# DarlingHang/st-nerf

Measured on NVIDIA H100. Metric: rays/sec, higher is better.
Workload: dtype f32 via fp16x3 split products (wgmma), f32 accumulate

## Files before the change

### st-nerf_b200/csrc/mlp_tc.cu

```cuda
#include <cuda_fp16.h>
#include <string.h>
#include <type_traits>
#include <vector>
#include "mlp_tc.cuh"
#include "resample.cuh"

namespace stnerf {

namespace {

constexpr int TILE_M = 128;
constexpr int ABLOCK = 16384;
constexpr int STAGE_BYTES = 16384;
constexpr int NTHREADS = 384;
constexpr int MATH_WG0 = 1, N_MATH_WARPS = 8;
constexpr int MAX_STAGE = 8;
constexpr int REGS_WG0 = 56, REGS_MATH = 224;
static_assert(128 * REGS_WG0 + 256 * REGS_MATH <= 384 * 168, "register file");
constexpr int BAR_WFULL = 0, BAR_WEMPTY = 8, BAR_RAWFULL = 16, BAR_RAWEMPTY = 18;
constexpr int MISC_ROWS = 256;
constexpr int MISC_PART = MISC_ROWS + 128 * 24;
constexpr int MISC_CDF = MISC_PART + 2048;
constexpr int MISC_TOTAL = MISC_CDF + 512;

__device__ __forceinline__ uint32_t smem_u32(const void* p) { return (uint32_t)__cvta_generic_to_shared(p); }

__device__ __forceinline__ void mbar_init(uint32_t bar, uint32_t count) {
  asm volatile("mbarrier.init.shared::cta.b64 [%0], %1;" ::"r"(bar), "r"(count) : "memory");
}
__device__ __forceinline__ void mbar_arrive(uint32_t bar) {
  asm volatile("mbarrier.arrive.shared::cta.b64 _, [%0];" ::"r"(bar) : "memory");
}
__device__ __forceinline__ void mbar_arrive_if(uint32_t bar, bool pred) {
  asm volatile("{\n\t.reg .pred p;\n\tsetp.ne.b32 p, %1, 0;\n\t@p mbarrier.arrive.shared::cta.b64 _, [%0];\n\t}" ::"r"(bar), "r"((uint32_t)pred)
               : "memory");
}
__device__ __forceinline__ void mbar_expect_tx(uint32_t bar, uint32_t bytes) {
  asm volatile("mbarrier.arrive.expect_tx.shared::cta.b64 _, [%0], %1;" ::"r"(bar), "r"(bytes) : "memory");
}
__device__ __forceinline__ void mbar_wait(uint32_t bar, uint32_t parity) {
  asm volatile(
      "{\n\t.reg .pred p;\n\t.reg .u32 c;\n\t"
      "mov.u32 c, 0;\n"
      "WAIT_%=:\n\t"
      "mbarrier.try_wait.parity.shared::cta.b64 p, [%0], %1;\n\t"
      "@p bra.uni DONE_%=;\n\t"
      "add.u32 c, c, 1;\n\t"
      "setp.gt.u32 p, c, 67108864;\n\t"
      "@p trap;\n\t"
      "bra.uni WAIT_%=;\n"
      "DONE_%=:\n\t}" ::"r"(bar), "r"(parity)
      : "memory");
}
__device__ __forceinline__ void bulk_g2s(uint32_t dst, const void* src, uint32_t bytes, uint32_t bar) {
  asm volatile("cp.async.bulk.shared::cluster.global.mbarrier::complete_tx::bytes [%0], [%1], %2, [%3];" ::"r"(dst),
               "l"(src), "r"(bytes), "r"(bar)
               : "memory");
}
__device__ __forceinline__ void fence_proxy_async() { asm volatile("fence.proxy.async.shared::cta;" ::: "memory"); }
template <int R>
__device__ __forceinline__ void setmaxnreg_dec() { asm volatile("setmaxnreg.dec.sync.aligned.u32 %0;" ::"n"(R)); }
template <int R>
__device__ __forceinline__ void setmaxnreg_inc() { asm volatile("setmaxnreg.inc.sync.aligned.u32 %0;" ::"n"(R)); }
__device__ __forceinline__ void wg_bar_sync(int wg) { asm volatile("bar.sync %0, 128;" ::"r"(1 + wg) : "memory"); }

__device__ __forceinline__ void load_stage_elect(uint32_t dst, const void* src, uint32_t bytes, uint32_t bar) {
  asm volatile(
      "{\n\t.reg .pred pe;\n\t"
      "elect.sync _|pe, 0xffffffff;\n\t"
      "@pe mbarrier.arrive.expect_tx.shared::cta.b64 _, [%3], %2;\n\t"
      "@pe cp.async.bulk.shared::cluster.global.mbarrier::complete_tx::bytes [%0], [%1], %2, [%3];\n\t}" ::"r"(dst),
      "l"(src), "r"(bytes), "r"(bar)
      : "memory");
}

__device__ __forceinline__ uint64_t desc_sw128(uint32_t saddr) {
  return (uint64_t)((saddr >> 4) & 0x3FFF) | ((uint64_t)1 << 16) | ((uint64_t)(1024 >> 4) << 32) | ((uint64_t)1 << 62);
}
__device__ __forceinline__ uint64_t desc_sw64(uint32_t saddr) {
  return (uint64_t)((saddr >> 4) & 0x3FFF) | ((uint64_t)1 << 16) | ((uint64_t)(512 >> 4) << 32) | ((uint64_t)2 << 62);
}
__device__ __forceinline__ void wgmma_fence() { asm volatile("wgmma.fence.sync.aligned;" ::: "memory"); }
__device__ __forceinline__ void wgmma_commit() { asm volatile("wgmma.commit_group.sync.aligned;" ::: "memory"); }
template <int N>
__device__ __forceinline__ void wgmma_wait() { asm volatile("wgmma.wait_group.sync.aligned %0;" ::"n"(N) : "memory"); }
template <int R>
__device__ __forceinline__ void acc_fence(float (&d)[128]) {
#pragma unroll
  for (int i = 0; i < R; ++i) asm volatile("" : "+f"(d[i])::"memory");
}

#define WGMMA_D_LO "%0, %1, %2, %3, %4, %5, %6, %7, %8, %9, %10, %11, %12, %13, %14, %15, %16, %17, %18, %19, %20, %21, %22, %23, %24, %25, %26, %27, %28, %29, %30, %31, %32, %33, %34, %35, %36, %37, %38, %39, %40, %41, %42, %43, %44, %45, %46, %47, %48, %49, %50, %51, %52, %53, %54, %55, %56, %57, %58, %59, %60, %61, %62, %63"
#define WGMMA_D_HI "%64, %65, %66, %67, %68, %69, %70, %71, %72, %73, %74, %75, %76, %77, %78, %79, %80, %81, %82, %83, %84, %85, %86, %87, %88, %89, %90, %91, %92, %93, %94, %95, %96, %97, %98, %99, %100, %101, %102, %103, %104, %105, %106, %107, %108, %109, %110, %111, %112, %113, %114, %115, %116, %117, %118, %119, %120, %121, %122, %123, %124, %125, %126, %127"
#define WGMMA_OPS_LO(d) \
    "+f"(d[0]), "+f"(d[1]), "+f"(d[2]), "+f"(d[3]), "+f"(d[4]), "+f"(d[5]), "+f"(d[6]), "+f"(d[7]), \
    "+f"(d[8]), "+f"(d[9]), "+f"(d[10]), "+f"(d[11]), "+f"(d[12]), "+f"(d[13]), "+f"(d[14]), "+f"(d[15]), \
    "+f"(d[16]), "+f"(d[17]), "+f"(d[18]), "+f"(d[19]), "+f"(d[20]), "+f"(d[21]), "+f"(d[22]), "+f"(d[23]), \
    "+f"(d[24]), "+f"(d[25]), "+f"(d[26]), "+f"(d[27]), "+f"(d[28]), "+f"(d[29]), "+f"(d[30]), "+f"(d[31]), \
    "+f"(d[32]), "+f"(d[33]), "+f"(d[34]), "+f"(d[35]), "+f"(d[36]), "+f"(d[37]), "+f"(d[38]), "+f"(d[39]), \
    "+f"(d[40]), "+f"(d[41]), "+f"(d[42]), "+f"(d[43]), "+f"(d[44]), "+f"(d[45]), "+f"(d[46]), "+f"(d[47]), \
    "+f"(d[48]), "+f"(d[49]), "+f"(d[50]), "+f"(d[51]), "+f"(d[52]), "+f"(d[53]), "+f"(d[54]), "+f"(d[55]), \
    "+f"(d[56]), "+f"(d[57]), "+f"(d[58]), "+f"(d[59]), "+f"(d[60]), "+f"(d[61]), "+f"(d[62]), "+f"(d[63])
#define WGMMA_OPS_HI(d) \
    "+f"(d[64]), "+f"(d[65]), "+f"(d[66]), "+f"(d[67]), "+f"(d[68]), "+f"(d[69]), "+f"(d[70]), "+f"(d[71]), \
    "+f"(d[72]), "+f"(d[73]), "+f"(d[74]), "+f"(d[75]), "+f"(d[76]), "+f"(d[77]), "+f"(d[78]), "+f"(d[79]), \
    "+f"(d[80]), "+f"(d[81]), "+f"(d[82]), "+f"(d[83]), "+f"(d[84]), "+f"(d[85]), "+f"(d[86]), "+f"(d[87]), \
    "+f"(d[88]), "+f"(d[89]), "+f"(d[90]), "+f"(d[91]), "+f"(d[92]), "+f"(d[93]), "+f"(d[94]), "+f"(d[95]), \
    "+f"(d[96]), "+f"(d[97]), "+f"(d[98]), "+f"(d[99]), "+f"(d[100]), "+f"(d[101]), "+f"(d[102]), "+f"(d[103]), \
    "+f"(d[104]), "+f"(d[105]), "+f"(d[106]), "+f"(d[107]), "+f"(d[108]), "+f"(d[109]), "+f"(d[110]), "+f"(d[111]), \
    "+f"(d[112]), "+f"(d[113]), "+f"(d[114]), "+f"(d[115]), "+f"(d[116]), "+f"(d[117]), "+f"(d[118]), "+f"(d[119]), \
    "+f"(d[120]), "+f"(d[121]), "+f"(d[122]), "+f"(d[123]), "+f"(d[124]), "+f"(d[125]), "+f"(d[126]), "+f"(d[127])

__device__ __forceinline__ void wgmma_n256(float (&d)[128], uint64_t da, uint64_t db) {
  asm volatile(
      "{\n\t.reg .pred p;\n\tsetp.ne.b32 p, %130, 0;\n\t"
      "wgmma.mma_async.sync.aligned.m64n256k16.f32.f16.f16 "
      "{" WGMMA_D_LO ", " WGMMA_D_HI "}, %128, %129, p, 1, 1, 0, 0;\n\t}"
      : WGMMA_OPS_LO(d), WGMMA_OPS_HI(d)
      : "l"(da), "l"(db), "r"(1));
}
__device__ __forceinline__ void wgmma_n128(float (&d)[128], uint64_t da, uint64_t db) {
  asm volatile(
      "{\n\t.reg .pred p;\n\tsetp.ne.b32 p, %66, 0;\n\t"
      "wgmma.mma_async.sync.aligned.m64n128k16.f32.f16.f16 "
      "{" WGMMA_D_LO "}, %64, %65, p, 1, 1, 0, 0;\n\t}"
      : WGMMA_OPS_LO(d)
      : "l"(da), "l"(db), "r"(1));
}
__device__ __forceinline__ void wgmma_n256_rs(float (&d)[128], const uint32_t* a, uint64_t db) {
  asm volatile(
      "{\n\t.reg .pred p;\n\tsetp.ne.b32 p, %133, 0;\n\t"
      "wgmma.mma_async.sync.aligned.m64n256k16.f32.f16.f16 "
      "{" WGMMA_D_LO ", " WGMMA_D_HI "}, {%128, %129, %130, %131}, %132, p, 1, 1, 0;\n\t}"
      : WGMMA_OPS_LO(d), WGMMA_OPS_HI(d)
      : "r"(a[0]), "r"(a[1]), "r"(a[2]), "r"(a[3]), "l"(db), "r"(1));
}
__device__ __forceinline__ void wgmma_n128_rs(float (&d)[128], const uint32_t* a, uint64_t db) {
  asm volatile(
      "{\n\t.reg .pred p;\n\tsetp.ne.b32 p, %69, 0;\n\t"
      "wgmma.mma_async.sync.aligned.m64n128k16.f32.f16.f16 "
      "{" WGMMA_D_LO "}, {%64, %65, %66, %67}, %68, p, 1, 1, 0;\n\t}"
      : WGMMA_OPS_LO(d)
      : "r"(a[0]), "r"(a[1]), "r"(a[2]), "r"(a[3]), "l"(db), "r"(1));
}

template <int N>
__device__ __forceinline__ void wgmma_k16(float (&d)[128], uint64_t da, uint64_t db) {
  if (N == 256) wgmma_n256(d, da, db);
  else wgmma_n128(d, da, db);
}
template <int N>
__device__ __forceinline__ void wgmma_k16_rs(float (&d)[128], const uint32_t* a, uint64_t db) {
  if (N == 256) wgmma_n256_rs(d, a, db);
  else wgmma_n128_rs(d, a, db);
}

__device__ __forceinline__ uint32_t pack_f16x2(float a, float b) {
  uint32_t r;
  asm("cvt.rn.satfinite.f16x2.f32 %0, %1, %2;" : "=r"(r) : "f"(b), "f"(a));
  return r;
}
__device__ __forceinline__ float2 unpack_f16x2(uint32_t p) {
  return __half22float2(*reinterpret_cast<const __half2*>(&p));
}

__host__ __device__ inline uint32_t sw128_offset(int row, int col) {
  return (uint32_t)((row >> 3) * 1024 + (row & 7) * 128 + ((((col >> 3) ^ (row & 7)) & 7) << 4) + ((col & 7) << 1));
}
__host__ __device__ inline uint32_t sw64_offset(int row, int col) {
  return (uint32_t)((row >> 3) * 512 + (row & 7) * 64 + ((((col >> 3) ^ ((row >> 1) & 3)) & 3) << 4) + ((col & 7) << 1));
}

enum { NET_SPACE = 0, NET_MOTION = 1 };

template <int NET> struct Sched;
template <> struct Sched<NET_SPACE> {
  static constexpr int N_LAYERS = 8;
  static constexpr bool lo_in_regs = true;
  static constexpr int act_base = 0, enc_base = 4 * ABLOCK;
  static constexpr int ENC_LO_STRIDE = ABLOCK;
  static constexpr int n_stage = 7, stage_bytes = STAGE_BYTES;
  static constexpr int ring_base = 6 * ABLOCK, misc_base = ring_base + n_stage * stage_bytes, smem_total = misc_base + MISC_TOTAL;
  static_assert(smem_total <= 232448, "shared memory budget (227 KB per CTA)");
  __host__ __device__ static constexpr int n_out(int l) { return l == 7 ? 128 : 256; }
  __host__ __device__ static constexpr int act_chunks(int l) { return l == 0 ? 0 : 4; }
  __host__ __device__ static constexpr int enc_chunks(int l) { return (l == 0 || l == 4) ? 1 : 0; }
  __host__ __device__ static constexpr bool enc_first(int l) { return l == 4; }
};
template <> struct Sched<NET_MOTION> {
  static constexpr int N_LAYERS = 5;
  static constexpr bool lo_in_regs = false;
  static constexpr int act_base = 0, enc_base = 0;
  static constexpr int LO_STRIDE = 2 * ABLOCK;
  static constexpr int ENC_LO_STRIDE = 2 * ABLOCK;
  static constexpr int n_stage = 8, stage_bytes = 8192;
  static constexpr int ring_base = 4 * ABLOCK, misc_base = ring_base + n_stage * stage_bytes, smem_total = misc_base + MISC_TOTAL;
  __host__ __device__ static constexpr int n_out(int) { return 128; }
  __host__ __device__ static constexpr int act_chunks(int l) { return l == 0 ? 0 : 2; }
  __host__ __device__ static constexpr int enc_chunks(int l) { return l == 0 ? 2 : 0; }
  __host__ __device__ static constexpr bool enc_first(int) { return false; }
};
static_assert(Sched<NET_SPACE>::n_stage <= MAX_STAGE && Sched<NET_MOTION>::n_stage <= MAX_STAGE, "barrier slots");

enum { A_HI = 0, A_LO = 1, A_HI_LO = 2 };
template <int A>
struct WStep {
  static constexpr int a = A;
  uint32_t offset;
  uint32_t sub;
};
template <int NET>
struct WSched {
  using S = Sched<NET>;
  __host__ __device__ static constexpr int n_chunks(int l) { return S::act_chunks(l) + S::enc_chunks(l); }
  __host__ __device__ static constexpr uint32_t stage_bytes(int l) { return (uint32_t)S::n_out(l) * 64; }
  __host__ __device__ static constexpr size_t layer_bytes(int l) { return (size_t)n_chunks(l) * 2  * 2  * stage_bytes(l); }
  __host__ __device__ static constexpr int chunk_at(int l, int c) {
    return S::enc_first(l) ? (c == 0 ? S::act_chunks(l) : c - 1) : c;
  }
  static constexpr bool enc_first_valid() {
    for (int l = 0; l < S::N_LAYERS; ++l)
      if (S::enc_first(l) && (S::act_chunks(l) == 0 || S::enc_chunks(l) == 0)) return false;
    return true;
  }
  static_assert(enc_first_valid(), "enc_first(l) needs activation chunks and an encoding chunk to reorder");
  template <bool LOFIRST, class C, class F>
  __device__ __forceinline__ static void for_each_step(int l, bool split, C&& chunk, F&& f) {
    const int nact = S::act_chunks(l), nch = nact + S::enc_chunks(l);
    const uint32_t bytes = stage_bytes(l);
    auto at = [&](const auto& a, int c, uint32_t sub, uint32_t lo_stage, auto op) {
      f(a, WStep<decltype(op)::value>{(2 * (2 * (uint32_t)c + sub) + lo_stage) * bytes, sub});
    };
    using HI = std::integral_constant<int, A_HI>;
    using LO = std::integral_constant<int, A_LO>;
    using HI_LO = std::integral_constant<int, A_HI_LO>;
    if (!LOFIRST || !split) {
      for (int c = 0; c < nch; ++c) {
        const auto a = chunk(chunk_at(l, c));
        for (uint32_t sub = 0; sub < 2; ++sub) {
          if (split) { at(a, c, sub, 1u, HI()); at(a, c, sub, 0u, HI_LO()); }
          else at(a, c, sub, 0u, HI());
        }
      }
    } else {
      for (int c = 0; c < nch; ++c) {
        const auto a = chunk(chunk_at(l, c));
        for (uint32_t sub = 0; sub < 2; ++sub) { at(a, c, sub, 1u, HI()); at(a, c, sub, 0u, LO()); }
      }
      for (int c = 0; c < nch; ++c) {
        const auto a = chunk(chunk_at(l, c));
        for (uint32_t sub = 0; sub < 2; ++sub) at(a, c, sub, 0u, HI());
      }
    }
  }
};

template <int NET>
__host__ __device__ constexpr size_t stream_bytes_per_tile() {
  size_t n = 0;
  for (int l = 0; l < Sched<NET>::N_LAYERS; ++l) n += WSched<NET>::layer_bytes(l);
  return n;
}

struct TcParams {
  FuseCoarse fuse;
  PointSrc src;
  const uint8_t* wstream;
  const float* aux;
  const float* cbuf;
  int exact;
  int single_last;
  int lo_first;
  float* raw;
  float* rgb_out;
  float* sigma_out;
  float* xyz_out;
  float* flow_out;
  const int* lerp_flag;
  int lerp_force;
};

constexpr int AUX_BIAS = 0, AUX_WSIG = 8 * 256, AUX_BSIG = AUX_WSIG + 256, AUX_WOUT = AUX_BSIG + 4,
              AUX_BOUT = AUX_WOUT + 3 * 128, AUX_FLOATS = AUX_BOUT + 4;


struct Pt { float x, y, z, tm; int out_index; int cidx; };

__device__ __forceinline__ Pt fetch_pt(const PointSrc& s, long long p, long long n_points) {
  Pt q;
  q.x = q.y = q.z = q.tm = 0.f;
  q.out_index = -1;
  q.cidx = 0;
  if (p >= n_points) return q;
  if (s.mode == SRC_EXPLICIT) {
    const float* pp = s.pos + p * s.pos_stride;
    q.x = pp[0]; q.y = pp[1]; q.z = pp[2];
    if (s.times) q.tm = s.times[p * s.time_stride];
    q.out_index = (int)p;
    q.cidx = (int)p;
    return q;
  }
  const long long slot = p / s.S;
  const int k = (int)(p - slot * s.S);
  const long long ray = s.hit ? (long long)s.hit[slot] : slot;
  const float* rp = s.rays + ray * s.ray_stride;
  q.tm = rp[6 + s.layer];
  q.out_index = (int)(ray * s.S + k);
  q.cidx = (int)slot;
  if (s.mode == SRC_XYZ) {
    q.x = s.pos[3 * p]; q.y = s.pos[3 * p + 1]; q.z = s.pos[3 * p + 2];
    return q;
  }
  if (s.mode == SRC_XYZ_MAP) {
    const int m = s.src_map[ray * s.S + k];
    const float* pp = (m < s.n_first) ? s.pos + 3 * (slot * s.n_first + m) : s.pos2 + 3 * (slot * (s.S - s.n_first) + (m - s.n_first));
    q.x = pp[0]; q.y = pp[1]; q.z = pp[2];
    return q;
  }
  const float tt = s.t[ray * s.S + k];
  float v[3] = {__fadd_rn(__fmul_rn(tt, rp[3]), rp[0]), __fadd_rn(__fmul_rn(tt, rp[4]), rp[1]),
                __fadd_rn(__fmul_rn(tt, rp[5]), rp[2])};
#pragma unroll
  for (int a = 0; a < 3; ++a) {
    if (s.shift_on) v[a] = __fsub_rn(v[a], s.shift[a]);
    if (s.scale_on) v[a] = __fadd_rn(__fdiv_rn(__fsub_rn(v[a], s.pivot[a]), s.scale), s.pivot[a]);
  }
  q.x = v[0]; q.y = v[1]; q.z = v[2];
  return q;
}

struct SinCos3 { float s0, s1, s2, c0, c1, c2; };
struct SinCos4 { float s0, s1, s2, s3, c0, c1, c2, c3; };
__device__ __noinline__ SinCos3 sincos_full3(float x0, float x1, float x2) {
  SinCos3 r;
  sincosf(x0, &r.s0, &r.c0); sincosf(x1, &r.s1, &r.c1); sincosf(x2, &r.s2, &r.c2);
  return r;
}
__device__ __noinline__ SinCos4 sincos_full4(float x0, float x1, float x2, float x3) {
  SinCos4 r;
  sincosf(x0, &r.s0, &r.c0); sincosf(x1, &r.s1, &r.c1); sincosf(x2, &r.s2, &r.c2); sincosf(x3, &r.s3, &r.c3);
  return r;
}

template <int NV>
__device__ __forceinline__ void store_row_split(uint8_t* hi_blk, int lo_stride, int row, int col0, const float (&v)[NV],
                                                bool exact) {
#pragma unroll
  for (int g = 0; g < NV / 8; ++g) {
    uint32_t hp[4], lp[4];
#pragma unroll
    for (int e = 0; e < 4; ++e) {
      const float a = v[g * 8 + 2 * e], b = v[g * 8 + 2 * e + 1];
      hp[e] = pack_f16x2(a, b);
      const float2 hf = unpack_f16x2(hp[e]);
      lp[e] = pack_f16x2(a - hf.x, b - hf.y);
    }
    const uint32_t off = sw128_offset(row, col0 + g * 8);
    *reinterpret_cast<uint4*>(hi_blk + off) = make_uint4(hp[0], hp[1], hp[2], hp[3]);
    if (exact) *reinterpret_cast<uint4*>(hi_blk + lo_stride + off) = make_uint4(lp[0], lp[1], lp[2], lp[3]);
  }
}

template <int half, int piece>
__device__ __forceinline__ void encode_space_piece(uint8_t* smem, const Pt& pt, int row, bool exact, float (&carry)[2]) {
  using S = Sched<NET_SPACE>;
  uint8_t* enc = smem + S::enc_base;
  const float xs[3] = {pt.x, pt.y, pt.z};
  float v[16];
  auto trig = [&](int f, float* dst) {
    const float fr = (float)(1 << f);
    const SinCos3 q = sincos_full3(xs[0] * fr, xs[1] * fr, xs[2] * fr);
    dst[0] = q.s0; dst[1] = q.s1; dst[2] = q.s2; dst[3] = q.c0; dst[4] = q.c1; dst[5] = q.c2;
  };
  if (piece == 0) {
    float t3[6];
    trig(5 * half + 0, v); trig(5 * half + 1, v + 6); trig(5 * half + 2, t3);
    v[12] = t3[0]; v[13] = t3[1]; v[14] = t3[2]; v[15] = t3[3];
    carry[0] = t3[4]; carry[1] = t3[5];
  } else {
    v[0] = carry[0]; v[1] = carry[1];
    trig(5 * half + 3, v + 2); trig(5 * half + 4, v + 8);
    v[14] = half == 0 ? xs[0] : xs[2];
    v[15] = half == 0 ? xs[1] : 0.f;
  }
  store_row_split<16>(enc, S::ENC_LO_STRIDE, row, half * 32 + piece * 16, v, exact);
}

template <int half, int piece>
__device__ __forceinline__ void encode_motion_piece(uint8_t* smem, const Pt& pt, int row, bool exact, bool lerp) {
  using S = Sched<NET_MOTION>;
  uint8_t* enc = smem + S::enc_base + half * ABLOCK;
  const float lo_t = floorf(pt.tm), wgt = pt.tm - lo_t, omw = 1.0f - wgt;
  const float in4[4] = {pt.x, pt.y, pt.z, pt.tm};
  auto trig = [&](int f, float* dst) {
    const float fr = (float)(1 << f);
    if (!lerp) {
      const SinCos4 q = sincos_full4(in4[0] * fr, in4[1] * fr, in4[2] * fr, in4[3] * fr);
      dst[0] = q.s0; dst[1] = q.s1; dst[2] = q.s2; dst[3] = q.s3; dst[4] = q.c0; dst[5] = q.c1; dst[6] = q.c2; dst[7] = q.c3;
    } else {
      const SinCos4 q = sincos_full4(in4[0] * fr, in4[1] * fr, in4[2] * fr, lo_t * fr);
      const SinCos3 q1 = sincos_full3((lo_t + 1.0f) * fr, 0.f, 0.f);
      const float s0[4] = {q.s0, q.s1, q.s2, q.s3}, c0[4] = {q.c0, q.c1, q.c2, q.c3};
      const float s1[4] = {q.s0, q.s1, q.s2, q1.s0}, c1[4] = {q.c0, q.c1, q.c2, q1.c0};
#pragma unroll
      for (int d = 0; d < 4; ++d) {
        dst[d] = __fadd_rn(__fmul_rn(omw, s0[d]), __fmul_rn(wgt, s1[d]));
        dst[4 + d] = __fadd_rn(__fmul_rn(omw, c0[d]), __fmul_rn(wgt, c1[d]));
      }
    }
  };
  float v[16];
  trig(5 * half + 2 * piece, v);
  if (piece < 2) {
    trig(5 * half + 2 * piece + 1, v + 8);
  } else {
#pragma unroll
    for (int d = 0; d < 4; ++d) {
      float a = 0.f;
      if (half == 0) {
        a = in4[d];
        if (lerp) {
          const float lo = d < 3 ? in4[d] : lo_t, hi = d < 3 ? in4[d] : lo_t + 1.0f;
          a = __fadd_rn(__fmul_rn(omw, lo), __fmul_rn(wgt, hi));
        }
      }
      v[8 + d] = a; v[12 + d] = 0.f;
    }
  }
  store_row_split<16>(enc, S::ENC_LO_STRIDE, row, piece * 16, v, exact);
}

template <int NET, int piece>
__device__ __forceinline__ void encode_piece(uint8_t* smem, const Pt& pt, int row, int half, bool exact, bool lerp,
                                             float (&carry)[2]) {
  if (NET == NET_SPACE) {
    if (half == 0) encode_space_piece<0, piece < 2 ? piece : 1>(smem, pt, row, exact, carry);
    else encode_space_piece<1, piece < 2 ? piece : 1>(smem, pt, row, exact, carry);
  } else {
    if (half == 0) encode_motion_piece<0, piece>(smem, pt, row, exact, lerp);
    else encode_motion_piece<1, piece>(smem, pt, row, exact, lerp);
  }
}

template <int NZ>
__device__ __noinline__ void fused_composite_loop(const TcParams& P, const float* rows, float* cdf, uint32_t bar_full, uint32_t bar_empty,
                                                  long long n_tiles, int j, int lane) {
  const FuseCoarse& F = P.fuse;
  const PointSrc& src = P.src;
  const long long n_slots = src.count ? (long long)(*src.count) : src.n_slots;
  const int n1 = 64, n2 = F.n2;
  uint32_t n = 0;
  for (long long tile = blockIdx.x; tile < n_tiles; tile += gridDim.x, ++n) {
    mbar_wait(bar_full, n & 1);
    const long long slot = tile * 2 + j;
    if (slot < n_slots) {
      const long long ray = src.hit ? (long long)src.hit[slot] : slot;
      const float* tp = src.t + ray * n1;
      const float4* rp = reinterpret_cast<const float4*>(rows) + j * 64;
      float t[2], sg[2];
#pragma unroll
      for (int s = 0; s < 2; ++s) {
        const int k = s * 32 + lane;
        const float tk = __ldg(tp + k);
        float v = rp[k].w;
        if (F.is_bkgd) {
          if (tk < F.near_plane) v = 0.0f;
        } else {
          if (tk < 0.0f) v = 0.0f;
          if (F.apply_thr && v < F.thr) v = 0.0f;
        }
        t[s] = tk;
        sg[s] = v;
      }
      const float* up = F.u ? F.u + ray * n2 : nullptr;
      const uint64_t seed = F.seed;
      const uint32_t stream = 64u + (uint32_t)F.layer;
      const unsigned long long gid = F.idmap(F.ray_base + ray);
      rs::LayerOut lo;
      rs::composite_resample_ray<2, NZ>(
          t, sg, n1, n2, F.boarder,
          [rp, lane](int s) {
            const float4 v = rp[s * 32 + lane];
            return make_float3(__fdiv_rn(1.0f, __fadd_rn(1.0f, expf(-v.x))), __fdiv_rn(1.0f, __fadd_rn(1.0f, expf(-v.y))),
                               __fdiv_rn(1.0f, __fadd_rn(1.0f, expf(-v.z))));
          },
          [up, seed, stream, gid](int jj) { return up ? up[jj] : philox_uniform(seed, stream, gid, (uint32_t)jj); },
          cdf, F.t_fine + ray * (n1 + n2), lane, lo, F.z_new ? F.z_new + ray * n2 : nullptr,
          F.z_new ? F.src_map + ray * (n1 + n2) : nullptr);
      if (F.img && lane < 5) {
        const long long rg = F.ray_base + ray;
        const float v = lane == 0 ? lo.pix[0] : lane == 1 ? lo.pix[1] : lane == 2 ? lo.pix[2] : lane == 3 ? lo.pix[3] : lo.pix[4];
        if (F.pixels) F.img[rg * 5 + lane] = v;
        else if (lane < 3) F.img[rg * 3 + lane] = v;
        else F.img[(long long)lane * F.n_total + rg] = v;
      }
    }
    __syncwarp();
    if (lane == 0) mbar_arrive(bar_empty);
  }
}

template <int NET, int N, bool LOFIRST>
__device__ __forceinline__ void mma_layer(float (&acc)[128], const uint32_t (&alo)[64], int l, bool sp, uint32_t sbase,
                                          uint32_t a_row, uint32_t bars, uint32_t& cnt, int lane) {
  using S = Sched<NET>;
  using W = WSched<NET>;
  constexpr uint32_t NST = S::n_stage;
#pragma unroll
  for (int i = 0; i < N / 2; ++i) acc[i] = 0.f;
  acc_fence<N / 2>(acc);
  wgmma_fence();
  const int nact = S::act_chunks(l);
  int pend = -1;
  auto release = [&](int s) {
    __syncwarp();
    mbar_arrive_if(bars + 8u * (uint32_t)(BAR_WEMPTY + s), lane == 0);
  };
  auto a_block = [&](int ch) {
    uint32_t hi, lo = 0;
    int z = -1;
    if (ch < nact) {
      hi = sbase + S::act_base + ch * ABLOCK + a_row;
      if constexpr (S::lo_in_regs) z = ch;
      else lo = hi + S::LO_STRIDE;
    } else {
      hi = sbase + S::enc_base + (ch - nact) * ABLOCK + a_row;
      lo = hi + S::ENC_LO_STRIDE;
    }
    return make_int3((int)hi, (int)lo, z);
  };
  W::template for_each_step<LOFIRST>(l, sp, a_block, [&](const int3& a, auto st) {
    const uint32_t hi = (uint32_t)a.x + 64u * st.sub, lo = (uint32_t)a.y + 64u * st.sub;
    const uint32_t s = cnt % NST, n = cnt / NST;
    mbar_wait(bars + 8u * (BAR_WFULL + s), n & 1);
    const uint32_t w = sbase + S::ring_base + s * S::stage_bytes;
    auto mma_lo = [&]() {
      if (S::lo_in_regs && a.z >= 0) {
        const int q = 2 * a.z + (int)st.sub;
#pragma unroll
        for (int i = 0; i < 8; ++i)
          if (q == i) {
#pragma unroll
            for (int ks = 0; ks < 2; ++ks) wgmma_k16_rs<N>(acc, &alo[8 * i + 4 * ks], desc_sw64(w + ks * 32));
          }
      } else {
#pragma unroll
        for (int ks = 0; ks < 2; ++ks) wgmma_k16<N>(acc, desc_sw128(lo + ks * 32), desc_sw64(w + ks * 32));
      }
    };
    if constexpr (decltype(st)::a == A_LO) {
      mma_lo();
    } else {
#pragma unroll
      for (int ks = 0; ks < 2; ++ks) wgmma_k16<N>(acc, desc_sw128(hi + ks * 32), desc_sw64(w + ks * 32));
      if constexpr (decltype(st)::a == A_HI_LO) mma_lo();
    }
    wgmma_commit();
    wgmma_wait<1>();
    if (pend >= 0) release(pend);
    pend = (int)s;
    ++cnt;
  });
  wgmma_wait<0>();
  acc_fence<N / 2>(acc);
  release(pend);
}

template <int NET, int N, bool SIGMA>
__device__ __forceinline__ void epi_hidden(const float (&acc)[128], const float* __restrict__ bias, const float* __restrict__ wsig,
                                           uint8_t* smem, int r0, int cq, bool lo_too, float& sig0, float& sig1,
                                           uint32_t (&alo)[64]) {
  using S = Sched<NET>;
#pragma unroll
  for (int j = 0; j < N / 8; ++j) {
    const int col = 8 * j + cq;
    const float2 b = __ldg(reinterpret_cast<const float2*>(bias + col));
    const float v00 = fmaxf(acc[4 * j] + b.x, 0.f), v01 = fmaxf(acc[4 * j + 1] + b.y, 0.f);
    const float v10 = fmaxf(acc[4 * j + 2] + b.x, 0.f), v11 = fmaxf(acc[4 * j + 3] + b.y, 0.f);
    if (SIGMA) {
      const float2 w = __ldg(reinterpret_cast<const float2*>(wsig + col));
      sig0 = fmaf(v00, w.x, sig0); sig0 = fmaf(v01, w.y, sig0);
      sig1 = fmaf(v10, w.x, sig1); sig1 = fmaf(v11, w.y, sig1);
    }
    uint8_t* blk = smem + S::act_base + (col >> 6) * ABLOCK;
    const uint32_t o0 = sw128_offset(r0, col & 63), o1 = sw128_offset(r0 + 8, col & 63);
    const uint32_t h0 = pack_f16x2(v00, v01), h1 = pack_f16x2(v10, v11);
    *reinterpret_cast<uint32_t*>(blk + o0) = h0;
    *reinterpret_cast<uint32_t*>(blk + o1) = h1;
    const float2 f0 = unpack_f16x2(h0), f1 = unpack_f16x2(h1);
    const uint32_t l0 = pack_f16x2(v00 - f0.x, v01 - f0.y), l1 = pack_f16x2(v10 - f1.x, v11 - f1.y);
    if constexpr (S::lo_in_regs) {
      alo[2 * j] = l0;
      alo[2 * j + 1] = l1;
    } else if (lo_too) {
      *reinterpret_cast<uint32_t*>(blk + S::LO_STRIDE + o0) = l0;
      *reinterpret_cast<uint32_t*>(blk + S::LO_STRIDE + o1) = l1;
    }
  }
}

__device__ __forceinline__ float quad_sum(float v) {
  v += __shfl_xor_sync(0xffffffffu, v, 1);
  v += __shfl_xor_sync(0xffffffffu, v, 2);
  return v;
}

template <int NET, bool LOFIRST>
__global__ void __launch_bounds__(NTHREADS, 1) mlp_tc_kernel(const __grid_constant__ TcParams P) {
  using S = Sched<NET>;
  extern __shared__ __align__(1024) uint8_t smem[];
  const uint32_t sbase = smem_u32(smem);
  if ((sbase & 1023u) != 0) {
    if (threadIdx.x == 0) printf("stnerf mlp_tc: dynamic shared memory base %u is not 1024-byte aligned\n", sbase);
    __trap();
  }
  const uint32_t bars = sbase + S::misc_base;
  auto BAR = [bars](int i) { return bars + 8u * (uint32_t)i; };
  Pt* s_rows = reinterpret_cast<Pt*>(smem + S::misc_base + MISC_ROWS);
  float* s_part = reinterpret_cast<float*>(smem + S::misc_base + MISC_PART);

  const int tid = threadIdx.x, lane = tid & 31;
  const int warp = __shfl_sync(0xffffffffu, tid >> 5, 0);
  const int wgi = __shfl_sync(0xffffffffu, tid >> 7, 0);
  const bool exact = P.exact != 0;
  const bool single_last = P.single_last != 0;
  auto split = [&](int l) { return exact && !(single_last && l == S::N_LAYERS - 1); };
  const long long n_points = src_num_points(P.src);
  const long long n_tiles = (n_points + TILE_M - 1) / TILE_M;
  constexpr uint32_t NST = S::n_stage;
  if (tid == 0) {
    for (int i = 0; i < MAX_STAGE; ++i) { mbar_init(BAR(BAR_WFULL + i), 1); mbar_init(BAR(BAR_WEMPTY + i), N_MATH_WARPS); }
    for (int j = 0; j < 2; ++j) {
      mbar_init(BAR(BAR_RAWFULL + j), 4);
      mbar_init(BAR(BAR_RAWEMPTY + j), 1);
    }
    asm volatile("fence.mbarrier_init.release.cluster;" ::: "memory");
  }
  __syncthreads();

  if (wgi < MATH_WG0) {
    if constexpr (S::lo_in_regs) setmaxnreg_dec<REGS_WG0>();
    if (warp == 0) {
      using W = WSched<NET>;
      uint32_t cnt = 0;
      for (long long tile = blockIdx.x; tile < n_tiles; tile += gridDim.x) {
        const uint8_t* layer = P.wstream;
        for (int l = 0; l < S::N_LAYERS; ++l) {
          W::template for_each_step<LOFIRST>(l, split(l), [](int) { return 0; }, [&](int, auto st) {
            const uint32_t s = cnt % NST, n = cnt / NST;
            mbar_wait(BAR(BAR_WEMPTY + s), (n & 1) ^ 1);
            load_stage_elect(sbase + S::ring_base + s * S::stage_bytes, layer + st.offset, W::stage_bytes(l), BAR(BAR_WFULL + s));
            ++cnt;
          });
          layer += W::layer_bytes(l);
        }
      }
    } else if (NET == NET_SPACE && (warp == 2 || warp == 3)) {
      if (P.fuse.on) {
        const int j = warp - 2;
        float* cdf = reinterpret_cast<float*>(smem + S::misc_base + MISC_CDF) + j * 64;
        if (P.fuse.n2 <= 128)
          fused_composite_loop<4>(P, s_part, cdf, BAR(BAR_RAWFULL + j), BAR(BAR_RAWEMPTY + j), n_tiles, j, lane);
        else
          fused_composite_loop<8>(P, s_part, cdf, BAR(BAR_RAWFULL + j), BAR(BAR_RAWEMPTY + j), n_tiles, j, lane);
      }
    }
  } else {
    if constexpr (S::lo_in_regs) setmaxnreg_inc<REGS_MATH>();
    const int wg = wgi - MATH_WG0;
    const int wt = tid & 127;
    const int erow = wg * 64 + (wt & 63), ehalf = wt >> 6;
    const int r0 = wg * 64 + (wt >> 5) * 16 + (lane >> 2);
    const int cq = 2 * (lane & 3);
    const uint32_t a_row = (uint32_t)wg * 8u * 1024u;
    const float* bias_all = P.aux + AUX_BIAS;
    const bool lerp = (NET == NET_MOTION) && (P.lerp_force >= 0 ? (P.lerp_force != 0) : (P.lerp_flag && *P.lerp_flag != 0));
    const bool fused = (NET == NET_SPACE) && P.fuse.on;
    uint32_t cnt = 0, tile_no = 0;
    float acc[128];
    uint32_t alo[64];
#pragma unroll
    for (int i = 0; i < 64; ++i) alo[i] = 0u;
    for (long long tile = blockIdx.x; tile < n_tiles; tile += gridDim.x, ++tile_no) {
      wg_bar_sync(wg);
      const Pt cur = fetch_pt(P.src, tile * TILE_M + erow, n_points);
      if (ehalf == 0) s_rows[erow] = cur;
      float carry[2] = {0.f, 0.f};
      if (NET == NET_MOTION) {
        uint8_t* enc = smem + S::enc_base + ehalf * ABLOCK;
        for (int c = (ehalf == 0 ? 48 : 40); c < 64; c += 8) {
          const uint32_t off = sw128_offset(erow, c);
          *reinterpret_cast<uint4*>(enc + off) = make_uint4(0, 0, 0, 0);
          *reinterpret_cast<uint4*>(enc + S::ENC_LO_STRIDE + off) = make_uint4(0, 0, 0, 0);
        }
      }
      encode_piece<NET, 0>(smem, cur, erow, ehalf, exact, lerp, carry);
      encode_piece<NET, 1>(smem, cur, erow, ehalf, exact, lerp, carry);
      if (NET == NET_MOTION) encode_piece<NET, 2>(smem, cur, erow, ehalf, exact, lerp, carry);
      float sig0 = 0.f, sig1 = 0.f;
      for (int l = 0; l < S::N_LAYERS; ++l) {
        fence_proxy_async();
        wg_bar_sync(wg);
        const bool last = (l == S::N_LAYERS - 1);
        if (!last) {
          mma_layer<NET, (NET == NET_SPACE ? 256 : 128), LOFIRST>(acc, alo, l, split(l), sbase, a_row, bars, cnt, lane);
          if (NET == NET_SPACE && l == 6)
            epi_hidden<NET, 256, true>(acc, bias_all + l * 256, P.aux + AUX_WSIG, smem, r0, cq, split(l + 1), sig0, sig1, alo);
          else
            epi_hidden<NET, (NET == NET_SPACE ? 256 : 128), false>(acc, bias_all + l * 256, nullptr, smem, r0, cq, split(l + 1), sig0,
                                                                  sig1, alo);
          continue;
        }
        mma_layer<NET, 128, LOFIRST>(acc, alo, l, split(l), sbase, a_row, bars, cnt, lane);
        const Pt p0 = s_rows[r0], p1 = s_rows[r0 + 8];
        const float* b0 = (NET == NET_SPACE) ? (P.cbuf + (size_t)p0.cidx * 128) : bias_all + l * 256;
        const float* b1 = (NET == NET_SPACE) ? (P.cbuf + (size_t)p1.cidx * 128) : bias_all + l * 256;
        float d0[3] = {0.f, 0.f, 0.f}, d1[3] = {0.f, 0.f, 0.f};
#pragma unroll
        for (int j = 0; j < 16; ++j) {
          const int col = 8 * j + cq;
          const float2 ba = __ldg(reinterpret_cast<const float2*>(b0 + col));
          const float2 bb = __ldg(reinterpret_cast<const float2*>(b1 + col));
          const float v00 = fmaxf(acc[4 * j] + ba.x, 0.f), v01 = fmaxf(acc[4 * j + 1] + ba.y, 0.f);
          const float v10 = fmaxf(acc[4 * j + 2] + bb.x, 0.f), v11 = fmaxf(acc[4 * j + 3] + bb.y, 0.f);
#pragma unroll
          for (int o = 0; o < 3; ++o) {
            const float2 w = __ldg(reinterpret_cast<const float2*>(P.aux + AUX_WOUT + o * 128 + col));
            d0[o] = fmaf(v00, w.x, d0[o]); d0[o] = fmaf(v01, w.y, d0[o]);
            d1[o] = fmaf(v10, w.x, d1[o]); d1[o] = fmaf(v11, w.y, d1[o]);
          }
        }
#pragma unroll
        for (int o = 0; o < 3; ++o) { d0[o] = quad_sum(d0[o]) + P.aux[AUX_BOUT + o]; d1[o] = quad_sum(d1[o]) + P.aux[AUX_BOUT + o]; }
        if (NET == NET_SPACE) { sig0 = quad_sum(sig0) + P.aux[AUX_BSIG]; sig1 = quad_sum(sig1) + P.aux[AUX_BSIG]; }
        if (fused) {
          if (tile_no > 0) mbar_wait(BAR(BAR_RAWEMPTY + wg), (tile_no - 1) & 1);
          if ((lane & 3) == 0) {
            reinterpret_cast<float4*>(s_part)[r0] = make_float4(d0[0], d0[1], d0[2], sig0);
            reinterpret_cast<float4*>(s_part)[r0 + 8] = make_float4(d1[0], d1[1], d1[2], sig1);
          }
          __syncwarp();
          if (lane == 0) mbar_arrive(BAR(BAR_RAWFULL + wg));
        }
        if ((lane & 3) == 0) {
#pragma unroll
          for (int h = 0; h < 2; ++h) {
            const Pt& p = h ? p1 : p0;
            const float* o = h ? d1 : d0;
            const float sg = h ? sig1 : sig0;
            if (p.out_index < 0) continue;
            const int oi = p.out_index;
            if (NET == NET_SPACE) {
              if (P.raw) reinterpret_cast<float4*>(P.raw)[oi] = make_float4(o[0], o[1], o[2], sg);
              if (P.rgb_out) { P.rgb_out[3 * (size_t)oi] = o[0]; P.rgb_out[3 * (size_t)oi + 1] = o[1]; P.rgb_out[3 * (size_t)oi + 2] = o[2]; }
              if (P.sigma_out) P.sigma_out[oi] = sg;
            } else {
              const long long pidx = tile * TILE_M + r0 + 8 * h;
              if (P.flow_out) { P.flow_out[3 * pidx] = o[0]; P.flow_out[3 * pidx + 1] = o[1]; P.flow_out[3 * pidx + 2] = o[2]; }
              if (P.xyz_out) {
                P.xyz_out[3 * pidx] = __fadd_rn(p.x, o[0]);
                P.xyz_out[3 * pidx + 1] = __fadd_rn(p.y, o[1]);
                P.xyz_out[3 * pidx + 2] = __fadd_rn(p.z, o[2]);
              }
            }
          }
        }
      }
    }
  }
}

constexpr int HB_SLOTS = 8;
__global__ void __launch_bounds__(128) head_bias_kernel(PointSrc src, const float* __restrict__ w_tail ,
                                                        const float* __restrict__ b1, int use_time,
                                                        float* __restrict__ cbuf) {
  __shared__ float s_enc[HB_SLOTS][48];
  const long long n_slots = src.count ? (long long)(*src.count) : src.n_slots;
  const int nk = PE_DIR + (use_time ? PE_TIME : 0);
  const int tid = threadIdx.x;
  float w[48];
#pragma unroll
  for (int k = 0; k < 48; ++k) w[k] = (k < nk) ? __ldg(w_tail + k * 128 + tid) : 0.f;
  const float bias = __ldg(b1 + tid);
  for (long long s0 = (long long)blockIdx.x * HB_SLOTS; s0 < n_slots; s0 += (long long)gridDim.x * HB_SLOTS) {
    __syncthreads();
    for (int e = tid; e < HB_SLOTS * 48; e += 128) {
      const int sl = e / 48, j = e - sl * 48;
      const long long slot = s0 + sl;
      float v = 0.f;
      if (slot < n_slots && j < nk) {
        float d[3], tm;
        if (src.mode == SRC_EXPLICIT) {
          d[0] = src.dirs[3 * slot]; d[1] = src.dirs[3 * slot + 1]; d[2] = src.dirs[3 * slot + 2];
          tm = src.times ? src.times[slot * src.time_stride] : 0.f;
        } else {
          const long long ray = src.hit ? (long long)src.hit[slot] : slot;
          const float* rp = src.rays + ray * src.ray_stride;
          d[0] = rp[3]; d[1] = rp[4]; d[2] = rp[5];
          tm = rp[6 + src.layer];
        }
        if (j < PE_DIR) {
          if (j < 3) v = d[j];
          else {
            const int r = j - 3, f = r / 6, m = r - 6 * f;
            const float a = d[m % 3] * (float)(1 << f);
            v = (m < 3) ? sinf(a) : cosf(a);
          }
        } else {
          const int r = j - PE_DIR;
          if (r == 0) v = tm;
          else {
            const int f = (r - 1) >> 1;
            const float a = tm * (float)(1 << f);
            v = ((r - 1) & 1) ? cosf(a) : sinf(a);
          }
        }
        v = fmaxf(v, 0.f);
      }
      s_enc[sl][j] = v;
    }
    __syncthreads();
#pragma unroll
    for (int sl = 0; sl < HB_SLOTS; ++sl) {
      const long long slot = s0 + sl;
      if (slot >= n_slots) break;
      float acc = bias;
#pragma unroll
      for (int k = 0; k < 48; ++k) acc = fmaf(w[k], s_enc[sl][k], acc);
      cbuf[slot * 128 + tid] = acc;
    }
  }
}

__global__ void __launch_bounds__(256, 1) wgmma_selftest_kernel(const float* __restrict__ A, const uint8_t* __restrict__ Bstages,
                                                               float* __restrict__ D, int reps) {
  extern __shared__ __align__(1024) uint8_t smem[];
  const uint32_t sbase = smem_u32(smem);
  const uint32_t bar = sbase + ABLOCK + 2 * STAGE_BYTES;
  const int tid = threadIdx.x, wg = tid >> 7, wt = tid & 127, lane = tid & 31;
  if ((sbase & 1023u) != 0) __trap();
  if (tid == 0) {
    mbar_init(bar, 1);
    asm volatile("fence.mbarrier_init.release.cluster;" ::: "memory");
  }
  if (tid < 128) {
    for (int c0 = 0; c0 < 64; c0 += 32) {
      float v[32];
      for (int i = 0; i < 32; ++i) v[i] = A[tid * 64 + c0 + i];
      store_row_split<32>(smem, 0, tid, c0, v, false);
    }
  }
  fence_proxy_async();
  __syncthreads();
  if (tid == 0) {
    mbar_expect_tx(bar, 2 * STAGE_BYTES);
    bulk_g2s(sbase + ABLOCK, Bstages, 2 * STAGE_BYTES, bar);
  }
  mbar_wait(bar, 0);
  float acc[128];
#pragma unroll
  for (int i = 0; i < 128; ++i) acc[i] = 0.f;
  acc_fence<128>(acc);
  wgmma_fence();
  for (int rep = 0; rep < reps; ++rep) {
#pragma unroll
    for (int sub = 0; sub < 2; ++sub)
#pragma unroll
// ... 273 lines not shown
```

Measured before the change: 748,800.

## Move space-net positional encoding to a producer warp and store epilogue via stmatrix

For the space network, a dedicated warp in the producer warpgroup now computes the positional encoding and sample rows for each tile. It is handed off to the math warpgroups through a full/empty mbarrier pair and double-buffered row storage, so the sin/cos work can overlap the MMA layers instead of stalling them. The hidden-layer epilogue now writes fp16 activations with stmatrix.x4 instead of scalar 32-bit swizzled stores. The cost is that a single warp (32 lanes) must encode 128 rows per tile, which could become the bottleneck. The encoding buffer is also released after layer 4's MMA, so correctness depends on that ordering.

Result: faster. 768,900 (median of 6 runs) (+2.7%).

```diff
diff --git a/st-nerf_b200/csrc/mlp_tc.cu b/st-nerf_b200/csrc/mlp_tc.cu
--- a/st-nerf_b200/csrc/mlp_tc.cu
+++ b/st-nerf_b200/csrc/mlp_tc.cu
@@ -17,9 +17,11 @@
 constexpr int MAX_STAGE = 8;
 constexpr int REGS_WG0 = 56, REGS_MATH = 224;
 static_assert(128 * REGS_WG0 + 256 * REGS_MATH <= 384 * 168, "register file");
-constexpr int BAR_WFULL = 0, BAR_WEMPTY = 8, BAR_RAWFULL = 16, BAR_RAWEMPTY = 18;
-constexpr int MISC_ROWS = 256;
-constexpr int MISC_PART = MISC_ROWS + 128 * 24;
+constexpr int BAR_WFULL = 0, BAR_WEMPTY = 8, BAR_RAWFULL = 16, BAR_RAWEMPTY = 18, BAR_ENCFULL = 20, BAR_ENCEMPTY = 21;
+constexpr int MISC_BARS = 32;
+constexpr int MISC_ROWS = 8 * MISC_BARS;
+static_assert(BAR_ENCEMPTY < MISC_BARS, "barrier slots");
+constexpr int MISC_PART = MISC_ROWS + 2 * 128 * 24;
 constexpr int MISC_CDF = MISC_PART + 2048;
 constexpr int MISC_TOTAL = MISC_CDF + 512;
 
@@ -167,6 +169,12 @@
 __host__ __device__ inline uint32_t sw128_offset(int row, int col) {
   return (uint32_t)((row >> 3) * 1024 + (row & 7) * 128 + ((((col >> 3) ^ (row & 7)) & 7) << 4) + ((col & 7) << 1));
 }
+__device__ __forceinline__ void stmatrix_x4(uint32_t addr, uint32_t r0, uint32_t r1, uint32_t r2, uint32_t r3) {
+  asm volatile("stmatrix.sync.aligned.m8n8.x4.shared.b16 [%0], {%1, %2, %3, %4};" ::"r"(addr), "r"(r0), "r"(r1), "r"(r2),
+               "r"(r3)
+               : "memory");
+}
+
 __host__ __device__ inline uint32_t sw64_offset(int row, int col) {
   return (uint32_t)((row >> 3) * 512 + (row & 7) * 64 + ((((col >> 3) ^ ((row >> 1) & 3)) & 3) << 4) + ((col & 7) << 1));
 }
@@ -186,7 +194,14 @@
   __host__ __device__ static constexpr int act_chunks(int l) { return l == 0 ? 0 : 4; }
   __host__ __device__ static constexpr int enc_chunks(int l) { return (l == 0 || l == 4) ? 1 : 0; }
   __host__ __device__ static constexpr bool enc_first(int l) { return l == 4; }
+  static constexpr int last_enc_layer = 4;
+  static constexpr bool last_enc_valid() {
+    for (int l = last_enc_layer + 1; l < N_LAYERS; ++l)
+      if (enc_chunks(l) != 0) return false;
+    return enc_chunks(last_enc_layer) != 0;
+  }
 };
+static_assert(Sched<NET_SPACE>::last_enc_valid(), "last_enc_layer must be the last layer with an encoding chunk");
 template <> struct Sched<NET_MOTION> {
   static constexpr int N_LAYERS = 5;
   static constexpr bool lo_in_regs = false;
@@ -331,11 +346,12 @@
 
 struct SinCos3 { float s0, s1, s2, c0, c1, c2; };
 struct SinCos4 { float s0, s1, s2, s3, c0, c1, c2, c3; };
-__device__ __noinline__ SinCos3 sincos_full3(float x0, float x1, float x2) {
+__device__ __forceinline__ SinCos3 sincos3_body(float x0, float x1, float x2) {
   SinCos3 r;
   sincosf(x0, &r.s0, &r.c0); sincosf(x1, &r.s1, &r.c1); sincosf(x2, &r.s2, &r.c2);
   return r;
 }
+__device__ __noinline__ SinCos3 sincos_full3(float x0, float x1, float x2) { return sincos3_body(x0, x1, x2); }
 __device__ __noinline__ SinCos4 sincos_full4(float x0, float x1, float x2, float x3) {
   SinCos4 r;
   sincosf(x0, &r.s0, &r.c0); sincosf(x1, &r.s1, &r.c1); sincosf(x2, &r.s2, &r.c2); sincosf(x3, &r.s3, &r.c3);
@@ -361,7 +377,7 @@
   }
 }
 
-template <int half, int piece>
+template <int half, int piece, bool INLINE_TRIG = false>
 __device__ __forceinline__ void encode_space_piece(uint8_t* smem, const Pt& pt, int row, bool exact, float (&carry)[2]) {
   using S = Sched<NET_SPACE>;
   uint8_t* enc = smem + S::enc_base;
@@ -369,7 +385,7 @@
   float v[16];
   auto trig = [&](int f, float* dst) {
     const float fr = (float)(1 << f);
-    const SinCos3 q = sincos_full3(xs[0] * fr, xs[1] * fr, xs[2] * fr);
+    const SinCos3 q = INLINE_TRIG ? sincos3_body(xs[0] * fr, xs[1] * fr, xs[2] * fr) : sincos_full3(xs[0] * fr, xs[1] * fr, xs[2] * fr);
     dst[0] = q.s0; dst[1] = q.s1; dst[2] = q.s2; dst[3] = q.c0; dst[4] = q.c1; dst[5] = q.c2;
   };
   if (piece == 0) {
@@ -500,6 +516,28 @@
   }
 }
 
+__device__ __noinline__ void encode_loop(const TcParams& P, uint8_t* smem, Pt* rows, uint32_t bar_full, uint32_t bar_empty,
+                                         long long n_tiles, long long n_points, bool exact, int lane) {
+  uint32_t n = 0;
+  for (long long tile = blockIdx.x; tile < n_tiles; tile += gridDim.x, ++n) {
+    if (n > 0) mbar_wait(bar_empty, (n - 1) & 1);
+    Pt* tr = rows + (n & 1) * TILE_M;
+#pragma unroll 1
+    for (int r = lane; r < TILE_M; r += 32) {
+      const Pt pt = fetch_pt(P.src, tile * TILE_M + r, n_points);
+      tr[r] = pt;
+      float carry[2] = {0.f, 0.f};
+      encode_space_piece<0, 0, true>(smem, pt, r, exact, carry);
+      encode_space_piece<0, 1, true>(smem, pt, r, exact, carry);
+      encode_space_piece<1, 0, true>(smem, pt, r, exact, carry);
+      encode_space_piece<1, 1, true>(smem, pt, r, exact, carry);
+    }
+    fence_proxy_async();
+    __syncwarp();
+    if (lane == 0) mbar_arrive(bar_full);
+  }
+}
+
 template <int NET, int N, bool LOFIRST>
 __device__ __forceinline__ void mma_layer(float (&acc)[128], const uint32_t (&alo)[64], int l, bool sp, uint32_t sbase,
                                           uint32_t a_row, uint32_t bars, uint32_t& cnt, int lane) {
@@ -568,35 +606,45 @@
 
 template <int NET, int N, bool SIGMA>
 __device__ __forceinline__ void epi_hidden(const float (&acc)[128], const float* __restrict__ bias, const float* __restrict__ wsig,
-                                           uint8_t* smem, int r0, int cq, bool lo_too, float& sig0, float& sig1,
-                                           uint32_t (&alo)[64]) {
+                                           uint32_t stm, bool lo_too, float& sig0, float& sig1, uint32_t (&alo)[64]) {
   using S = Sched<NET>;
 #pragma unroll
-  for (int j = 0; j < N / 8; ++j) {
-    const int col = 8 * j + cq;
-    const float2 b = __ldg(reinterpret_cast<const float2*>(bias + col));
-    const float v00 = fmaxf(acc[4 * j] + b.x, 0.f), v01 = fmaxf(acc[4 * j + 1] + b.y, 0.f);
-    const float v10 = fmaxf(acc[4 * j + 2] + b.x, 0.f), v11 = fmaxf(acc[4 * j + 3] + b.y, 0.f);
-    if (SIGMA) {
-      const float2 w = __ldg(reinterpret_cast<const float2*>(wsig + col));
-      sig0 = fmaf(v00, w.x, sig0); sig0 = fmaf(v01, w.y, sig0);
-      sig1 = fmaf(v10, w.x, sig1); sig1 = fmaf(v11, w.y, sig1);
-    }
-    uint8_t* blk = smem + S::act_base + (col >> 6) * ABLOCK;
-    const uint32_t o0 = sw128_offset(r0, col & 63), o1 = sw128_offset(r0 + 8, col & 63);
-    const uint32_t h0 = pack_f16x2(v00, v01), h1 = pack_f16x2(v10, v11);
-    *reinterpret_cast<uint32_t*>(blk + o0) = h0;
-    *reinterpret_cast<uint32_t*>(blk + o1) = h1;
-    const float2 f0 = unpack_f16x2(h0), f1 = unpack_f16x2(h1);
-    const uint32_t l0 = pack_f16x2(v00 - f0.x, v01 - f0.y), l1 = pack_f16x2(v10 - f1.x, v11 - f1.y);
-    if constexpr (S::lo_in_regs) {
-      alo[2 * j] = l0;
-      alo[2 * j + 1] = l1;
-    } else if (lo_too) {
-      *reinterpret_cast<uint32_t*>(blk + S::LO_STRIDE + o0) = l0;
-      *reinterpret_cast<uint32_t*>(blk + S::LO_STRIDE + o1) = l1;
-    }
-  }
+  for (int j = 0; j < N / 8; j += 2) {
+    uint32_t h[4], lw[4];
+#pragma unroll
+    for (int e = 0; e < 2; ++e) {
+      const int jj = j + e;
+      const float2 b = __ldg(reinterpret_cast<const float2*>(bias + 8 * jj));
+      const float v00 = fmaxf(acc[4 * jj] + b.x, 0.f), v01 = fmaxf(acc[4 * jj + 1] + b.y, 0.f);
+      const float v10 = fmaxf(acc[4 * jj + 2] + b.x, 0.f), v11 = fmaxf(acc[4 * jj + 3] + b.y, 0.f);
+      if (SIGMA) {
+        const float2 w = __ldg(reinterpret_cast<const float2*>(wsig + 8 * jj));
+        sig0 = fmaf(v00, w.x, sig0); sig0 = fmaf(v01, w.y, sig0);
+        sig1 = fmaf(v10, w.x, sig1); sig1 = fmaf(v11, w.y, sig1);
+      }
+      const uint32_t h0 = pack_f16x2(v00, v01), h1 = pack_f16x2(v10, v11);
+      const float2 f0 = unpack_f16x2(h0), f1 = unpack_f16x2(h1);
+      const uint32_t l0 = pack_f16x2(v00 - f0.x, v01 - f0.y), l1 = pack_f16x2(v10 - f1.x, v11 - f1.y);
+      h[2 * e] = h0; h[2 * e + 1] = h1;
+      lw[2 * e] = l0; lw[2 * e + 1] = l1;
+      if constexpr (S::lo_in_regs) {
+        alo[2 * jj] = l0;
+        alo[2 * jj + 1] = l1;
+      }
+    }
+    const uint32_t addr = (stm ^ ((uint32_t)(j & 7) << 4)) + (uint32_t)(j >> 3) * ABLOCK;
+    stmatrix_x4(addr, h[0], h[1], h[2], h[3]);
+    if constexpr (!S::lo_in_regs) {
+      if (lo_too) stmatrix_x4(addr + S::LO_STRIDE, lw[0], lw[1], lw[2], lw[3]);
+    }
+  }
+}
+
+template <int NET>
+__device__ __forceinline__ uint32_t epi_row_address(uint32_t sbase, int wg, int wt, int lane) {
+  static_assert(Sched<NET>::act_base % 1024 == 0, "activation blocks must keep the 1024-byte swizzle alignment");
+  const int row = wg * 64 + (wt >> 5) * 16 + 8 * ((lane >> 3) & 1) + (lane & 7);
+  return sbase + (uint32_t)Sched<NET>::act_base + sw128_offset(row, 8 * (lane >> 4));
 }
 
 __device__ __forceinline__ float quad_sum(float v) {
@@ -634,6 +682,8 @@
       mbar_init(BAR(BAR_RAWFULL + j), 4);
       mbar_init(BAR(BAR_RAWEMPTY + j), 1);
     }
+    mbar_init(BAR(BAR_ENCFULL), 1);
+    mbar_init(BAR(BAR_ENCEMPTY), N_MATH_WARPS);
     asm volatile("fence.mbarrier_init.release.cluster;" ::: "memory");
   }
   __syncthreads();
@@ -655,6 +705,8 @@
           layer += W::layer_bytes(l);
         }
       }
+    } else if (NET == NET_SPACE && warp == 1) {
+      encode_loop(P, smem, s_rows, BAR(BAR_ENCFULL), BAR(BAR_ENCEMPTY), n_tiles, n_points, exact, lane);
     } else if (NET == NET_SPACE && (warp == 2 || warp == 3)) {
       if (P.fuse.on) {
         const int j = warp - 2;
@@ -673,6 +725,7 @@
     const int r0 = wg * 64 + (wt >> 5) * 16 + (lane >> 2);
     const int cq = 2 * (lane & 3);
     const uint32_t a_row = (uint32_t)wg * 8u * 1024u;
+    const uint32_t stm = epi_row_address<NET>(sbase, wg, wt, lane);
     const float* bias_all = P.aux + AUX_BIAS;
     const bool lerp = (NET == NET_MOTION) && (P.lerp_force >= 0 ? (P.lerp_force != 0) : (P.lerp_flag && *P.lerp_flag != 0));
     const bool fused = (NET == NET_SPACE) && P.fuse.on;
@@ -683,20 +736,23 @@
     for (int i = 0; i < 64; ++i) alo[i] = 0u;
     for (long long tile = blockIdx.x; tile < n_tiles; tile += gridDim.x, ++tile_no) {
       wg_bar_sync(wg);
-      const Pt cur = fetch_pt(P.src, tile * TILE_M + erow, n_points);
-      if (ehalf == 0) s_rows[erow] = cur;
-      float carry[2] = {0.f, 0.f};
-      if (NET == NET_MOTION) {
+      const Pt* rows = s_rows + (NET == NET_SPACE ? (tile_no & 1) * TILE_M : 0);
+      if constexpr (NET == NET_SPACE) {
+        mbar_wait(BAR(BAR_ENCFULL), tile_no & 1);
+      } else {
+        const Pt cur = fetch_pt(P.src, tile * TILE_M + erow, n_points);
+        if (ehalf == 0) s_rows[erow] = cur;
+        float carry[2] = {0.f, 0.f};
         uint8_t* enc = smem + S::enc_base + ehalf * ABLOCK;
         for (int c = (ehalf == 0 ? 48 : 40); c < 64; c += 8) {
           const uint32_t off = sw128_offset(erow, c);
           *reinterpret_cast<uint4*>(enc + off) = make_uint4(0, 0, 0, 0);
           *reinterpret_cast<uint4*>(enc + S::ENC_LO_STRIDE + off) = make_uint4(0, 0, 0, 0);
         }
-      }
-      encode_piece<NET, 0>(smem, cur, erow, ehalf, exact, lerp, carry);
-      encode_piece<NET, 1>(smem, cur, erow, ehalf, exact, lerp, carry);
-      if (NET == NET_MOTION) encode_piece<NET, 2>(smem, cur, erow, ehalf, exact, lerp, carry);
+        encode_piece<NET, 0>(smem, cur, erow, ehalf, exact, lerp, carry);
+        encode_piece<NET, 1>(smem, cur, erow, ehalf, exact, lerp, carry);
+        encode_piece<NET, 2>(smem, cur, erow, ehalf, exact, lerp, carry);
+      }
       float sig0 = 0.f, sig1 = 0.f;
       for (int l = 0; l < S::N_LAYERS; ++l) {
         fence_proxy_async();
@@ -704,15 +760,18 @@
         const bool last = (l == S::N_LAYERS - 1);
         if (!last) {
           mma_layer<NET, (NET == NET_SPACE ? 256 : 128), LOFIRST>(acc, alo, l, split(l), sbase, a_row, bars, cnt, lane);
+          if constexpr (NET == NET_SPACE) {
+            if (l == S::last_enc_layer) mbar_arrive_if(BAR(BAR_ENCEMPTY), lane == 0);
+          }
           if (NET == NET_SPACE && l == 6)
-            epi_hidden<NET, 256, true>(acc, bias_all + l * 256, P.aux + AUX_WSIG, smem, r0, cq, split(l + 1), sig0, sig1, alo);
+            epi_hidden<NET, 256, true>(acc, bias_all + l * 256 + cq, P.aux + AUX_WSIG + cq, stm, split(l + 1), sig0, sig1, alo);
           else
-            epi_hidden<NET, (NET == NET_SPACE ? 256 : 128), false>(acc, bias_all + l * 256, nullptr, smem, r0, cq, split(l + 1), sig0,
+            epi_hidden<NET, (NET == NET_SPACE ? 256 : 128), false>(acc, bias_all + l * 256 + cq, nullptr, stm, split(l + 1), sig0,
                                                                   sig1, alo);
           continue;
         }
         mma_layer<NET, 128, LOFIRST>(acc, alo, l, split(l), sbase, a_row, bars, cnt, lane);
-        const Pt p0 = s_rows[r0], p1 = s_rows[r0 + 8];
+        const Pt p0 = rows[r0], p1 = rows[r0 + 8];
         const float* b0 = (NET == NET_SPACE) ? (P.cbuf + (size_t)p0.cidx * 128) : bias_all + l * 256;
         const float* b1 = (NET == NET_SPACE) ? (P.cbuf + (size_t)p1.cidx * 128) : bias_all + l * 256;
         float d0[3] = {0.f, 0.f, 0.f}, d1[3] = {0.f, 0.f, 0.f};
```
